# peabody124/PosePipeline

Measured on AMD Instinct MI355X. Metric: frames/sec (whole node), detect->2D->3D cascade on 1080p; MPJPE vs reference, higher is better.
Workload: dtype f32; eligible float32 convolutions are evaluated as 2-term float16 splits (22 significand bits under per-channel / per-sample power-of-two scales, 3 products per term) on the 16-bit matrix cores with float32 accumulation (float32-accurate at any input magnitude, not bit-identical: tests/test_gpu_spl

## Files before the change

### include/posepipe_hip.h

```cpp
#ifndef POSEPIPE_HIP_H
#define POSEPIPE_HIP_H

#include <stddef.h>
#include <stdint.h>

#ifdef __cplusplus
extern "C" {
#endif

#define PP_ABI_VERSION 10

typedef enum {
    PP_OK = 0,
    PP_ERR_ARG = -1,
    PP_ERR_HIP = -2,
    PP_ERR_STATE = -3,
    PP_ERR_UNSUPPORTED = -4
} pp_status;

typedef enum { PP_MEM_HOST = 0, PP_MEM_DEVICE = 1 } pp_mem_kind;

typedef struct pp_ctx pp_ctx;
typedef struct pp_net pp_net;
typedef struct pp_tracker pp_tracker;
// ... 70 lines not shown
    int32_t up2_log2, up3_log2;
} pp_op;

typedef struct pp_buf {
    int32_t h, w, c;
    int32_t pad;
} pp_buf;

int pp_net_create(pp_ctx* ctx, const pp_op* ops, int n_ops, const pp_buf* bufs, int n_bufs,
                  const float* weights, size_t n_weights, int max_batch, pp_net** out);
int pp_net_create_mem(pp_ctx* ctx, const pp_op* ops, int n_ops, const pp_buf* bufs, int n_bufs,
                      const float* weights, size_t n_weights, int weights_mem, int max_batch, pp_net** out);
#define PP_NET_NUMERICS_DEFAULT 0
#define PP_NET_NUMERICS_EXACT 1
#define PP_NET_NUMERICS_SPLIT 2
#define PP_NET_NUMERICS_SPLIT_BF16 3
#define PP_NET_NUMERICS_SPLIT_F16 4
int pp_net_create_ex(pp_ctx* ctx, const pp_op* ops, int n_ops, const pp_buf* bufs, int n_bufs,
                     const float* weights, size_t n_weights, int weights_mem, int max_batch, int numerics, pp_net** out);
int pp_net_numerics(pp_net* net);
int pp_net_split_kind(pp_net* net);
void pp_net_destroy(pp_net* net);
int pp_net_buffer(pp_net* net, int buf, void** dptr, size_t* bytes_per_sample);
int pp_net_input_amax(pp_net* net, int buf, void** dptr);
int pp_net_run(pp_net* net, int batch, int first_op, int last_op);
int pp_net_forward(pp_net* net, int batch, int in_buf, const float* in, int out_buf, float* out,
                   int mem);
int pp_net_set_lanes(pp_net* net, int enable);
int pp_net_set_lane_count(pp_net* net, int n_lanes);
int pp_net_capture(pp_net* net, int batch);
int pp_net_profile(pp_net* net, int batch, float* ms_per_op);
int pp_net_conv_kinds(pp_net* net, int* kinds);
int pp_net_folded_into(pp_net* net, int* into);

int pp_conv_force(int ct, int pt);
int pp_conv_variant(int variant);
int pp_conv_exact(int exact);
int pp_conv_split_kind(int f16);

int pp_conv2d(pp_ctx* ctx, const pp_op* op, int n, int hin, int win, const float* x,
              const float* w, const float* bias, const float* res1, const float* res2, float* y,
              int res1_h, int res1_w, int mem);

int pp_crop_resize_bilinear(pp_ctx* ctx, const float* src_nhwc4, int n_src, int src_h, int src_w, const int32_t* rects5, int n,
                            int out_h, int out_w, float* out_nhwc4);

int pp_net_vit_timing(pp_net* net, int enable, float* ms3, int* n_gemm);
int pp_f32_to_bf16(pp_ctx* ctx, const float* x, uint16_t* y, size_t n);
int pp_gemm_bf16(pp_ctx* ctx, const uint16_t* a, const uint16_t* w, const float* bias, const float* res, int res_mod,
                 void* c, int m, int n, int k, int act, int out_bf16);
int pp_layernorm(pp_ctx* ctx, const float* x, const float* gamma, const float* beta, int rows, int dim, float eps,
                 void* y, int out_bf16);
int pp_attention_bf16(pp_ctx* ctx, const uint16_t* qkv, int batch, int tokens, int heads, int head_dim, uint16_t* out);

int pp_crop_affine_normalize(pp_ctx* ctx, const uint8_t* frames, int n_frames, int h, int w,
                             const int32_t* frame_idx, const double* bbox_tlwh, int n_person,
                             int out_w, int out_h, const float* lut, const int32_t* chan_map,
                             int flip, float* out, float* center_scale, uint8_t* crop_u8,
                             int32_t* valid, int mem);

int pp_flip_merge_decode(pp_ctx* ctx, const float* hm, const float* hm_flip, int n, int k, int h,
                         int w, const int32_t* flip_perm, int shift_heatmap, int post,
                         int blur_kernel, const float* center_scale, float* kpts, float* merged,
                         int mem);

int pp_topdown_create(pp_net* net, int in_buf, int out_buf, int num_joints, const int32_t* flip_perm,
// ... 136 lines not shown
```

### posepipeline_amd/csrc/conv_split.hip

```cpp
#include <algorithm>
#include <atomic>
#include <map>
#include <mutex>
#include <type_traits>
#include <vector>
#include <cstring>
#include <cstdio>

#include "pp_internal.h"
#include "pp_amax.h"

#ifndef PP_SPLIT_ABLATE
#define PP_SPLIT_ABLATE 0
#endif

typedef __attribute__((ext_vector_type(8))) __bf16 bf16x8;
typedef __attribute__((ext_vector_type(8))) _Float16 f16x8;
typedef __attribute__((ext_vector_type(16))) float f32x16;

std::atomic<int> g_split_gemm_epi{-1};

namespace {


struct SplitArgs {
    const float* x;
    const uint4* w;
    const float* bias;
    const float* res1;
    const float* res2;
    float* y;
    int N, H, W, Cin, Cout, ncb;
    int xp_h, xp_w;
    int y_pad, r1_pad, r2_pad, relu;
    int nchunks;
    int tiles_x, tiles_y, TH, TW, bw_log2, gx_log2;
    int PWp;
    int NP, NPp;
    int mode, stride;
    int r1_shift, r1_H, r1_W;
    int ktaps, KW, pad, Hin, Win;
    long long S;
    unsigned x_bytes;
    int xcd_remap;
    int SP;
    int gx, gy;
    int col_major;
    int epi_lds;
    unsigned dv_per[2], dv_row[2];
    unsigned dv_tx[2], dv_ty[2], dv_pw[2];
    unsigned dv_ncol[2], dv_run0[2], dv_run1[2];
    unsigned dv_ktaps[2], dv_kw[2];
    const float* wscale;
    const unsigned* x_amax;
    unsigned* y_amax;
    const float* x2;
    const unsigned* x2_amax;
    int Cin2, stride2, xp2_h, xp2_w, seg1;
#ifdef PP_SPLIT_TIMELINE
    unsigned long long* dbg;
#endif
};

#ifdef PP_SPLIT_TIMELINE
#define PP_TL_DECL unsigned long long tl_t[10] = {0, 0, 0, 0, 0, 0, 0, 0, 0, 0}
#define PP_TL_MARK(i) do { if (a.dbg) tl_t[i] = __builtin_amdgcn_s_memtime(); } while (0)
#define PP_TL_FLUSH()                                                                                                    \
    do {                                                                                                                 \
        if (a.dbg && threadIdx.x == 0) {                                                                                 \
            unsigned hw, xcc;                                                                                            \
            asm volatile("s_getreg_b32 %0, hwreg(HW_REG_HW_ID)" : "=s"(hw));                                            \
            asm volatile("s_getreg_b32 %0, hwreg(HW_REG_XCC_ID)" : "=s"(xcc));                                          \
            unsigned long long* r = a.dbg + (size_t)blockIdx.x * 16;                                                     \
            r[0] = blockIdx.x; r[1] = ((unsigned long long)xcc << 32) | hw;                                              \
            r[2] = tl_t[0]; r[3] = tl_t[1]; r[4] = tl_t[2]; r[5] = tl_t[3]; r[6] = L; r[7] = col;                       \
            for (int i_ = 4; i_ < 10; ++i_) r[4 + i_] = tl_t[i_];                                                        \
        }                                                                                                                \
    } while (0)
#else
#define PP_TL_DECL
#define PP_TL_MARK(i)
#define PP_TL_FLUSH()
// ... 60 lines not shown
        if (x > 20.f) return x;
        const double n = exp((double)x);
        const double t = n * (n + 2.0);
        return x * (float)(t / (t + 2.0));
    }
    if (act == PP_ACT_ELU) return x > 0.f ? x : (float)expm1((double)x);
    if (act == PP_ACT_SWISH) return x * (float)(1.0 / (1.0 + exp(-(double)x)));
    return x;
}

__device__ __forceinline__ int lane_q(int r) {
    const int g1 = ((r >= 4 && r < 12) || (r >= 16 && r < 20) || r >= 28) ? 1 : 0;
    int idx;
    if (!g1) idx = r < 4 ? r : r < 16 ? r - 8 : r - 12;
    else idx = r < 12 ? r - 4 : r < 20 ? r - 8 : r - 16;
    return g1 * 16 + idx;
}
__device__ __forceinline__ void block_pixel(int r, int bw_log2, int& iy, int& ix) {
    if (bw_log2 == 0) {
        iy = 0;
        ix = r;
        return;
    }
    const int q = lane_q(r);
    if (bw_log2 == 1) {
        iy = q >> 4;
        ix = q & 15;
    } else {
        iy = ((q >> 3) & 1) * 2 + (q >> 4);
        ix = q & 7;
    }
}

enum { MODE_TILE = 0, MODE_STREAM = 1, MODE_GEMM = 2 };

template <int T, int NSLOT, int COB, int PXB = 2, int NW = 4, bool RING4 = false, bool H = false, bool S2 = false>
__global__ __launch_bounds__(64 * NW, NW == 4 ? 2 : 1) void conv_split_kernel(SplitArgs a) {
    static_assert(!S2 || (T == 9 && RING4 && H && PXB == 1), "S2 is the 4-wave fp16 ring form with one pixel block per wave");
    constexpr int NT = 64 * NW;
    constexpr int XP = H ? 2 : 3;
    constexpr int WPL = H ? 2 : 3;
    constexpr bool WLDS = NW == 8 || RING4;
    static_assert(!RING4 || (NW == 4 && T == 9), "RING4 is the 4-wave 3x3 form");
    extern __shared__ __attribute__((aligned(16))) unsigned char smem[];
    const int tid = threadIdx.x;
    const int lane = tid & 63;
    const int wave = tid >> 6;
    unsigned L = blockIdx.x, col = blockIdx.y;
    PP_TL_DECL;
    PP_TL_MARK(0);
    if (a.xcd_remap) {
        if (!xcd_tile_column(blockIdx.x, a, L, col)) return;
    }
    const int cb0 = (int)col * COB;
    const int plane_bytes = 2 * a.NPp * 16;
    const int buf_bytes = XP * plane_bytes;

    int n = 0, x0 = 0, y0 = 0;
    unsigned s0 = 0;
    if (a.mode == MODE_TILE) {
        const unsigned L2 = pp_udiv(L, a.dv_tx);
        const int tx = (int)(L - L2 * (unsigned)a.tiles_x);
        n = (int)pp_udiv(L2, a.dv_ty);
        const int ty = (int)(L2 - (unsigned)n * (unsigned)a.tiles_y);
        x0 = tx * a.TW;
        y0 = ty * a.TH;
    } else {
        s0 = L * (unsigned)(32 * PXB * NW);
    }

    unsigned goff[NSLOT];
    unsigned vmask[T == 1 ? NSLOT : 1];
    int simg[H ? NSLOT : 1];
    const int woff0 = ((((tid & 3) >> 1) * a.NPp + (tid >> 2)) * 16 + (tid & 1) * 8);
    if (a.mode == MODE_STREAM) {
        const int pos0 = (int)s0 - a.PWp - 1 + (tid >> 2);
        const unsigned cin4 = (unsigned)a.Cin * 4u;
        const unsigned base = (unsigned)pos0 * cin4 + (unsigned)(tid & 3) * 16u;
#pragma unroll
        for (int j = 0; j < NSLOT; ++j) goff[j] = pos0 + (NT / 4) * j < 0 ? 0xffffffffu : base + (unsigned)((NT / 4) * j) * cin4;
        if constexpr (T == 1) {
#pragma unroll
            for (int j = 0; j < NSLOT; ++j) vmask[j] = 0;
        }
        if constexpr (H) {
#pragma unroll
            for (int j = 0; j < NSLOT; ++j) {
                const int pj = pos0 + (NT / 4) * j;
                simg[j] = (int)pp_udiv((unsigned)min(max(pj, 0), (int)a.S - 1), a.dv_per);
            }
        }
    } else {
#pragma unroll
    for (int j = 0; j < NSLOT; ++j) {
        const int u = tid + NT * j;
        const int p = u >> 2, quad = u & 3;
        const bool in_patch = p < a.NP;
        unsigned off = 0xffffffffu;
        if constexpr (H) simg[j] = n;
        if constexpr (S2) {
            const int ph = (int)pp_udiv((unsigned)p, a.dv_row), r = p - ph * a.SP;
            const int qr = (int)pp_udiv((unsigned)r, a.dv_pw), qc = r - qr * a.PWp;
            const int pr = 2 * qr + (ph >> 1), pc = 2 * qc + (ph & 1);
            const int iy = 2 * y0 - 1 + pr, ix = 2 * x0 - 1 + pc;
            if (in_patch && pc <= 2 * a.TW && (unsigned)iy < (unsigned)a.Hin && (unsigned)ix < (unsigned)a.Win)
                off = (unsigned)(((n * a.xp_h + iy) * a.xp_w + ix) * a.Cin) * 4u;
        } else if (a.mode == MODE_TILE) {
            const int pr = (int)pp_udiv((unsigned)p, a.dv_pw), pc = p - pr * a.PWp;
            const int iy = y0 - 1 + pr, ix = x0 - 1 + pc;
            if (in_patch && pc < a.TW + 2 && (unsigned)iy < (unsigned)a.H && (unsigned)ix < (unsigned)a.W)
                off = (unsigned)(((n * a.xp_h + iy) * a.xp_w + ix) * a.Cin) * 4u;
        } else {
            const unsigned m = s0 + (unsigned)p;
            if constexpr (T == 1) vmask[j] = 0;
            if (in_patch && m < (unsigned)a.S) {
                const int img = (int)pp_udiv(m, a.dv_per), rem = (int)(m - (unsigned)img * (unsigned)(a.H * a.W));
                const int ho = (int)pp_udiv((unsigned)rem, a.dv_row), wo = rem - ho * a.W;
                if constexpr (H) simg[j] = img;
                if (T == 1 && a.ktaps > 1) {
                    const int iy0 = ho * a.stride - a.pad, ix0 = wo * a.stride - a.pad;
                    off = (unsigned)(((img * a.xp_h + iy0) * a.xp_w + ix0) * a.Cin) * 4u;
                    unsigned vm = 0;
// ... 80 lines not shown
    if constexpr (WLDS) {
        issue_w(0);
        issue_w(1);
        issue_w(2);
        load_patch(0);
    } else {
        load_patch(0);
        load_w(wf[0]);
    }
    unsigned xam[H ? NSLOT : 1];
    if constexpr (H) {
#pragma unroll
        for (int j = 0; j < NSLOT; ++j) xam[j] = a.x_amax[simg[j]];
    }
    __builtin_amdgcn_sched_barrier(0);

    auto pixel_coords = [&](int lane_, int wave_, int pb, int& aofs_, int& on_, int& oy_, int& ox_, bool& ok_) {
        if (a.mode == MODE_TILE) {
            const int BW = 32 >> a.bw_log2, BH = 1 << a.bw_log2;
            int by, bx;
            block_pixel(lane_ & 31, a.bw_log2, by, bx);
            const int b = wave_ * PXB + pb;
            const int gy = b >> a.gx_log2, gx = b & ((1 << a.gx_log2) - 1);
            const int ry = gy * BH + by, rx = gx * BW + bx;
            aofs_ = (((lane_ >> 5) * a.NPp) + ry * a.PWp + rx) * 16;
            on_ = n;
            oy_ = y0 + ry;
            ox_ = x0 + rx;
            ok_ = oy_ < a.H && ox_ < a.W;
        } else {
            const unsigned per = a.mode == MODE_STREAM ? (unsigned)(a.xp_h * a.PWp) : (unsigned)(a.H * a.W);
            const unsigned row = a.mode == MODE_STREAM ? (unsigned)a.PWp : (unsigned)a.W;
            const int pl = (wave_ * PXB + pb) * 32 + (lane_ & 31);
            aofs_ = (((lane_ >> 5) * a.NPp) + pl) * 16;
            const unsigned sp = s0 + (unsigned)pl;
            const bool in = sp < (unsigned)a.S;
            const unsigned sc = in ? sp : 0u;
            const unsigned img = pp_udiv(sc, a.dv_per);
            const unsigned rem = sc - img * per;
            const unsigned yy = pp_udiv(rem, a.dv_row);
            on_ = (int)img;
            oy_ = (int)yy;
            ox_ = (int)(rem - yy * row);
            ok_ = in && oy_ < a.H && ox_ < a.W;
        }
    };
    int aofs[PXB];
#pragma unroll
    for (int pb = 0; pb < PXB; ++pb) {
        int on_, oy_, ox_;
        bool ok_;
        pixel_coords(lane, wave, pb, aofs[pb], on_, oy_, ox_, ok_);
    }

    f32x16 acc[COB][PXB];
#pragma unroll
    for (int cb = 0; cb < COB; ++cb)
#pragma unroll
        for (int pb = 0; pb < PXB; ++pb)
#pragma unroll
            for (int i = 0; i < 16; ++i) acc[cb][pb][i] = 0.f;
    if constexpr (H) {
#pragma unroll
        for (int q = 0; q < (NSLOT + 3) / 4; ++q) sxe[q] = 0;
#pragma unroll
        for (int j = 0; j < NSLOT; ++j) sxe[j >> 2] |= pp_amax_exp(xam[j]) << (8 * (j & 3));
    }

    auto load_x = [&](const unsigned char* pbuf, int t, int pb) {
        const int dy = t / 3, dx = t % 3;
        const int toff = S2 ? ((((dy & 1) * 2 + (dx & 1)) * a.SP) + (dy >> 1) * a.PWp + (dx >> 1)) * 16 : T == 9 ? (dy * a.PWp + dx) * 16 : 0;
#pragma unroll
        for (int pl = 0; pl < XP; ++pl) xf[pb][pl] = *reinterpret_cast<const uint4*>(pbuf + pl * plane_bytes + aofs[pb] + toff);
    };

    if constexpr (!WLDS) {
        store_patch(0, 0, NSLOT);
// ... 1525 lines not shown
}

__global__ __launch_bounds__(256) void split_weights_stem7_kernel(const float* w, uint4* out, int CoutPad, const float* cmax) {
    const int i = blockIdx.x * 256 + threadIdx.x;
    if (i >= STEM_STEPS * 2 * 64) return;
    const int lane = i & 63, cb = (i >> 6) & 1, s = i >> 7;
    const int cout = cb * 32 + (lane & 31);
    unsigned short h[2][8];
#pragma unroll
    for (int j = 0; j < 8; ++j) {
        const int dy = s >> 1, dx = 4 * (s & 1) + 2 * (lane >> 5) + (j >> 2), c = j & 3;
        float v = 0.f;
        if (dx < 7) {
            const int k = (dy * 7 + dx) * 4 + c;
            v = w[((size_t)(k >> 5) * CoutPad + cout) * 32 + 8 * (k & 3) + ((k & 31) >> 2)];
        }
        unsigned short q2;
        split_weight_h(v, channel_scale(cmax[cout]), h[0][j], h[1][j], q2);
    }
#pragma unroll
    for (int pn = 0; pn < 2; ++pn) {
        uint4 o;
        o.x = h[pn][0] | ((unsigned)h[pn][1] << 16);
        o.y = h[pn][2] | ((unsigned)h[pn][3] << 16);
        o.z = h[pn][4] | ((unsigned)h[pn][5] << 16);
        o.w = h[pn][6] | ((unsigned)h[pn][7] << 16);
        out[(size_t)(((s * 2 + cb) * 2 + pn) * 64 + lane)] = o;
    }
}

}


static TileGeom tap_tiling(const ConvArgs& a, int nw, int stream_env) {
    const int max_np = nw == 8 ? 768 : 512, xp_h = a.Hin + a.x_pad, xp_w = a.Win + a.x_pad;
    TileGeom g = pick_tile(a.Hout, a.Wout, max_np, nw / 2);
    g.mode = MODE_TILE;
    const int snp = 64 * nw + 2 + 2 * xp_w;
    const double stream_eff = (double)a.Hout * a.Wout / ((double)xp_h * xp_w);
    bool use_stream = a.x_pad >= 1 && snp <= max_np && (g.eff < 0 || stream_eff > g.eff + 0.02);
    if (stream_env == 0 && g.eff >= 0) use_stream = false;
    if (stream_env == 1 && a.x_pad >= 1 && snp <= max_np) use_stream = true;
    if (use_stream) {
        g.mode = MODE_STREAM;
        g.PWp = xp_w;
        g.NP = g.NPp = snp;
        while (g.NPp % 8 != 4) ++g.NPp;
    }
    return g;
}

SplitPlan pp_conv_split_plan(const ConvArgs& a) {
    static const int stem7_on = env_int("POSEPIPE_SPLIT_STEM7", 1);
    static const int s2_on = env_int("POSEPIPE_SPLIT_S2", 1), s2p_on = env_int("POSEPIPE_SPLIT_S2P", 1);
    static const int gemm8_on = env_int("POSEPIPE_SPLIT_GEMM8", 1), gemm4_min_c = env_int("POSEPIPE_SPLIT_GEMM4_MIN_C", 64);
    static const int gemm_min_cin = env_int("POSEPIPE_SPLIT_GEMM_MIN_CIN", 1024);
    static const int c48_on = env_int("POSEPIPE_SPLIT_C48", 1), c48_mult = env_int("POSEPIPE_SPLIT_C48_MULT", 0);
    static const int stream_env = env_int("POSEPIPE_SPLIT_STREAM", -1);
    const char* s2_env = getenv("POSEPIPE_SPLIT_S2_MIN_CIN");
    SplitPlan p;
    p.f16 = a.split_f16 != 0;
    const size_t wpl = p.f16 ? 2 : 3;
    p.ncb = (a.Cout + 31) / 32;
    p.nout = p.ncb * 32;
    if (stem7_on && p.f16 && a.KH == 7 && a.KW == 7 && a.stride == 2 && a.pad_h == 3 && a.pad_w == 3 && a.dil_h == 1 && a.dil_w == 1 &&
        a.Cin == 4 && a.Cout == 64 && a.CoutPad >= 64 && a.up_log2 == 0 && !a.out_nchw && !a.res1 && !a.res2 &&
        (a.relu == PP_RELU_NONE || a.relu == PP_RELU_FIRST || a.relu == PP_RELU_LAST) && (a.y_stride == 0 || a.y_stride == a.Cout) &&
        a.y_coff == 0 && a.Hout == (a.Hin - 1) / 2 + 1 && a.Wout == (a.Win - 1) / 2 + 1) {
        p.kernel = SPLIT_STEM7;
        p.cin = a.Cin;
        p.frag_bytes = STEM_WBYTES;
        p.bytes = p.frag_bytes + (size_t)2 * p.nout * sizeof(float);
        return p;
    }
    const bool k3 = a.KH == 3 && a.KW == 3 && a.stride == 1 && a.pad_h == 1 && a.pad_w == 1 && a.dil_h == 1 && a.dil_w == 1 &&
                    a.Hout == a.Hin && a.Wout == a.Win;
    const bool k1 = a.KH == 1 && a.KW == 1 && a.pad_h == 0 && a.pad_w == 0;
    const bool full = a.KH == a.Hin && a.KW == a.Win && a.pad_h == 0 && a.pad_w == 0 && a.dil_h == 1 && a.dil_w == 1 &&
                      a.x_pad == 0 && a.Hout == 1 && a.Wout == 1 && !k1;
    const bool s2_pick = s2_env ? a.Cin >= atoi(s2_env) : p.f16 ? (a.Cin >= 96 || (a.Cin >= 48 && p.ncb >= 6)) : (a.Cin >= 128 && (p.ncb & 1) == 0);
    const bool s2_shape = a.KH == 3 && a.KW == 3 && a.stride == 2 && a.pad_h == 1 && a.pad_w == 1 && a.dil_h == 1 && a.dil_w == 1 && !full;
    const bool s2p_map = a.Hout * a.Wout >= 1500 || (a.Hout * a.Wout >= 400 && a.Cout >= 96);
    const bool s2p = s2p_on && p.f16 && s2_shape && s2p_map;
    const bool k3s2 = s2_on && s2_shape && (s2_pick || s2p);
    if (!(k3 || k1 || full || k3s2)) return p;
    p.taps = (k3 || k3s2) ? 9 : 1;
    p.cin = full ? a.K : a.Cin;
    const bool product = gemm8_on && p.taps == 1 && p.cin >= gemm4_min_c && a.Cout % 128 == 0;
    const bool one_column = p.f16 && p.cin >= 256 && a.Cout > 32 && a.Cout <= 64 && a.HWout >= 4096;
    if (p.taps == 1 && p.cin < gemm_min_cin && !one_column && !product) return p;
    const bool res1_plain = !a.res1 || (a.res1_off_w == 0 && a.res1_shift >= 0 && a.res1_shift <= 4 &&
                                        ((a.Hout - 1) >> a.res1_shift) < a.res1_H && ((a.Wout - 1) >> a.res1_shift) < a.res1_W &&
                                        (a.res1_shift > 0 || (a.res1_H == a.Hout && a.res1_W == a.Wout)));
    if (!(p.cin % 16 == 0 && a.Cout % 4 == 0 && a.up_log2 == 0 && !a.out_nchw && res1_plain && a.relu <= PP_ACT_SWISH &&
          (a.y_stride == 0 || a.y_stride == a.Cout) && a.y_coff == 0))
        return p;
    const bool c48 = c48_on && k3 && ((a.Cout > 32 && a.Cout <= 48) || (c48_mult == 1 && a.Cout % 48 == 0) || (c48_mult == 2 && a.Cout == 192));
    if (a.Cin2 > 0) {
        if (!(product && p.f16 && k1 && a.stride == 1 && !a.res1 && a.Cin2 % 16 == 0 && a.stride2 >= 1 && a.x_pad == 0 && a.x2_pad == 0 &&
              (a.Hout - 1) * a.stride2 < a.Hin2 && (a.Wout - 1) * a.stride2 < a.Win2))
            return SplitPlan();
        p.cin2 = a.Cin2;
    }
    size_t steps = (size_t)((p.cin + p.cin2) / 16) * p.taps;
    if (product) {
        p.kernel = SPLIT_PRODUCT;
    } else if (!k3 && !s2p) {
        p.kernel = p.taps > 1 ? SPLIT_TAP_GATHER : SPLIT_ONE_TAP;
        p.tile[0].mode = MODE_GEMM;
        p.tile[0].NP = 256;
        p.tile[0].NPp = 260;
    } else if (s2p) {
        p.kernel = SPLIT_S2P;
        p.tile[0] = pick_tile_s2(a.Hout, a.Wout, 13 * 64);
        p.tile[0].mode = MODE_TILE;
    } else if (c48) {
        p.kernel = SPLIT_C48;
        p.ncb = (a.Cout + 47) / 48 * 3;
        p.nout = p.ncb * 16;
        steps = (size_t)(p.cin / 16) * 5;
        p.tile[0] = tap_tiling(a, 4, stream_env);
    } else {
        p.kernel = SPLIT_TAP3;
        p.tile[0] = tap_tiling(a, 4, stream_env);
        p.tile[1] = tap_tiling(a, 8, stream_env);
    }
    p.frag_bytes = (steps + 1) * p.ncb * wpl * 64 * sizeof(uint4);
    p.bytes = p.frag_bytes + (p.f16 ? (size_t)2 * p.nout * sizeof(float) : 0);
    if (p.cin2 > 0) {
        p.bias_off = (p.bytes + 15) / 16 * 16;
        p.bytes = p.bias_off + (size_t)a.CoutPad * sizeof(float);
    }
    return p;
}

static int split_weights_folded(const SplitPlan& p, const ConvArgs& a, void* out, hipStream_t stream) {
    const int kcat = p.cin + p.cin2, kpad = (kcat + 31) / 32 * 32;
    const size_t total = (size_t)kpad * a.CoutPad;
    float* cat = nullptr;
    PP_HIP_CHECK(hipMalloc((void**)&cat, total * sizeof(float)));
    hipLaunchKernelGGL(concat_weights_kernel, dim3((unsigned)((total + 255) / 256)), dim3(256), 0, stream, a.w, a.w2, cat, p.cin, p.cin2, a.CoutPad, total);
    SplitPlan q = p;
    q.cin = kcat;
    q.cin2 = 0;
    ConvArgs b = a;
    b.w = cat;
    b.Cin = kcat; b.K = kcat; b.Kpad = kpad;
    int rc = pp_conv_split_weights(q, b, out, stream);
    std::vector<float> b0(a.CoutPad), b1(a.CoutPad);
    hipError_t e = hipStreamSynchronize(stream);
    if (e == hipSuccess) e = hipMemcpy(b0.data(), a.bias, b0.size() * sizeof(float), hipMemcpyDeviceToHost);
    if (e == hipSuccess) e = hipMemcpy(b1.data(), a.bias2, b1.size() * sizeof(float), hipMemcpyDeviceToHost);
    for (size_t i = 0; i < b0.size(); ++i) b0[i] += b1[i];
    if (e == hipSuccess) e = hipMemcpy(static_cast<unsigned char*>(out) + p.bias_off, b0.data(), b0.size() * sizeof(float), hipMemcpyHostToDevice);
    (void)hipFree(cat);
    if (rc == PP_OK && e != hipSuccess) {
        pp_set_error("split_weights (folded shortcut) failed: %s", hipGetErrorString(e));
// ... 73 lines not shown
    if (!path || (only_cin && a.Cin != only_cin) || recorded >= max_launches) return nullptr;
    ++recorded;
    if (!tl_buf && hipMalloc(&tl_buf, TL_MAX_WG * 128) != hipSuccess) return nullptr;
    (void)hipMemsetAsync(tl_buf, 0, TL_MAX_WG * 128, stream);
    return tl_buf;
}
static void tl_end(const ConvArgs& a, const SplitArgs& s, const char* kernel, unsigned nwg, hipStream_t stream) {
    if (!s.dbg) return;
    (void)hipStreamSynchronize(stream);
    nwg = std::min<unsigned>(nwg, TL_MAX_WG);
    std::vector<unsigned long long> h((size_t)nwg * 16);
    (void)hipMemcpy(h.data(), tl_buf, h.size() * 8, hipMemcpyDeviceToHost);
    static int launch = 0;
    FILE* f = fopen(getenv("POSEPIPE_SPLIT_TIMELINE"), "ab");
    if (!f) return;
    long long hdr[16] = {0x54494d454c494e45ll, launch++, (long long)nwg, a.N, a.Hout, a.Wout, a.Cin, a.Cout, s.mode, s.nchunks, s.gx, s.gy,
                         a.res1 != nullptr, a.res2 != nullptr, 0, 0};
    memcpy(&hdr[14], kernel, std::min<size_t>(strlen(kernel), 15));
    fwrite(hdr, 8, 16, f);
    fwrite(h.data(), 8, h.size(), f);
    fclose(f);
}
#define PP_TL_BEGIN() s.dbg = tl_begin(a, stream)
#define PP_TL_END(name, nwg) tl_end(a, s, name, nwg, stream)
#else
#define PP_TL_BEGIN()
#define PP_TL_END(name, nwg)
#endif

static void fill_divisors(SplitArgs& s) {
    const bool stream_mode = s.mode == MODE_STREAM;
    make_magic(stream_mode ? (unsigned)(s.xp_h * s.PWp) : (unsigned)(s.H * s.W), s.dv_per);
    make_magic(stream_mode ? (unsigned)s.PWp : (unsigned)s.W, s.dv_row);
    make_magic((unsigned)std::max(s.tiles_x, 1), s.dv_tx);
    make_magic((unsigned)std::max(s.tiles_y, 1), s.dv_ty);
    make_magic((unsigned)std::max(s.PWp, 1), s.dv_pw);
    make_magic((unsigned)std::max(s.gy, 1), s.dv_ncol);
    make_magic((unsigned)std::max(s.gx >> 3, 1), s.dv_run0);
    make_magic((unsigned)((s.gx >> 3) + 1), s.dv_run1);
    make_magic((unsigned)std::max(s.ktaps, 1), s.dv_ktaps);
    make_magic((unsigned)std::max(s.KW, 1), s.dv_kw);
}

template <auto K, int MAX_LDS, class Args>
static void launch_split(dim3 grid, unsigned threads, size_t lds, hipStream_t stream, const Args& s) {
    static PpPerDeviceOnce once;
    once.run([] { (void)hipFuncSetAttribute((const void*)K, hipFuncAttributeMaxDynamicSharedMemorySize, MAX_LDS); });
    hipLaunchKernelGGL(K, grid, dim3(threads), lds, stream, s);
}

template <int NS, int... MORE, class F>
static void with_nslot(int nslot, F&& f) {
    if constexpr (sizeof...(MORE) == 0) f(std::integral_constant<int, NS>());
    else if (nslot <= NS) f(std::integral_constant<int, NS>());
    else with_nslot<MORE...>(nslot, f);
}

template <int T, int NW, bool R4, int NS>
static void launch_tap(int cob, bool f16, dim3 grid, size_t lds, hipStream_t stream, const SplitArgs& s) {
    constexpr int L = (NW == 8 ? 160 : 100) * 1024;
    if constexpr (R4) {
        if (cob == 3) return launch_split<conv_split_kernel<9, NS, 3, 2, 4, true, true>, L>(grid, 256, lds, stream, s);
        if (cob == 4) return launch_split<conv_split_kernel<9, NS, 4, 2, 4, true, true>, L>(grid, 256, lds, stream, s);
    }
    if (f16 && cob == 2) launch_split<conv_split_kernel<T, NS, 2, 2, NW, R4, true>, L>(grid, 64 * NW, lds, stream, s);
    else if (f16) launch_split<conv_split_kernel<T, NS, 1, 2, NW, R4, true>, L>(grid, 64 * NW, lds, stream, s);
    else if (cob == 2) launch_split<conv_split_kernel<T, NS, 2, 2, NW, R4, false>, L>(grid, 64 * NW, lds, stream, s);
    else launch_split<conv_split_kernel<T, NS, 1, 2, NW, R4, false>, L>(grid, 64 * NW, lds, stream, s);
}

static unsigned apply_tiling(SplitArgs& s, const TileGeom& g, const ConvArgs& a, int nw) {
    s.mode = g.mode;
    s.NP = g.NP;
    s.NPp = g.NPp;
    if (g.mode == MODE_GEMM) {
        s.S = (long long)a.M;
        return (unsigned)((a.M + 255) / 256);
    }
    s.PWp = g.PWp;
    if (g.mode == MODE_STREAM) {
        s.S = (long long)a.N * s.xp_h * s.xp_w;
        return (unsigned)((s.S + 64 * nw - 1) / (64 * nw));
    }
    s.tiles_x = g.tiles_x; s.tiles_y = g.tiles_y; s.TH = g.TH; s.TW = g.TW; s.bw_log2 = g.bw_log2; s.gx_log2 = g.gx_log2;
    return (unsigned)(g.tiles_x * g.tiles_y * a.N);
}

static int launch_stem7(const ConvArgs& a, hipStream_t stream) {
    if (!a.x_amax) {
        pp_set_error("conv_split: the fp16 form needs the per-sample maximum of its input (ConvArgs::x_amax)");
        return PP_ERR_STATE;
    }
    StemArgs s{};
    s.x = a.x; s.w = (const uint4*)a.wsplit; s.bias = a.bias; s.y = a.y;
    s.wscale = reinterpret_cast<const float*>(static_cast<const unsigned char*>(a.wsplit) + STEM_WBYTES);
    s.x_amax = a.x_amax; s.y_amax = a.y_amax;
    s.N = a.N; s.Hin = a.Hin; s.Win = a.Win; s.xp_h = a.Hin + a.x_pad; s.xp_w = a.Win + a.x_pad;
    s.Hout = a.Hout; s.Wout = a.Wout; s.y_pad = a.y_pad; s.relu = a.relu;
    s.tiles_x = (a.Wout + STEM_TW - 1) / STEM_TW;
    s.tiles_y = (a.Hout + STEM_TH - 1) / STEM_TH;
    s.ntiles = a.N * s.tiles_x * s.tiles_y;
    s.x_bytes = a.x_bytes;
    make_magic((unsigned)s.tiles_x, s.dv_tx);
    make_magic((unsigned)s.tiles_y, s.dv_ty);
    static const int ncu = [] {
        int dev = 0, n = 256;
        if (hipGetDevice(&dev) == hipSuccess) (void)hipDeviceGetAttribute(&n, hipDeviceAttributeMultiprocessorCount, dev);
        return n > 0 ? n : 256;
    }();
    launch_split<conv_split_stem7_kernel, STEM_LDS>(dim3((unsigned)std::min(s.ntiles, ncu)), 512, STEM_LDS, stream, s);
    hipError_t e = hipGetLastError();
    if (e != hipSuccess) {
        pp_set_error("conv_split_stem7 launch failed: %s", hipGetErrorString(e));
        return PP_ERR_HIP;
    }
    return PP_OK;
}

int pp_launch_conv_split(const SplitPlan& p, const ConvArgs& a, hipStream_t stream) {
    if (a.wsplit && p.kernel == SPLIT_STEM7) return launch_stem7(a, stream);
    if (!a.wsplit || p.kernel == SPLIT_NONE) {
        pp_set_error("conv_split: layer not eligible");
        return PP_ERR_ARG;
    }
    static const int colmaj_mb = env_int("POSEPIPE_SPLIT_COLMAJOR_MB", 256), gemm_remap = env_int("POSEPIPE_SPLIT_GEMM_REMAP", 1);
    static const int epi_env = env_int("POSEPIPE_SPLIT_GEMM_EPI", 1);
    static const int cob2_env = env_int("POSEPIPE_SPLIT_S2_COB", 0), cob_env = env_int("POSEPIPE_SPLIT_COB", 0);
    static const int nw8_f16 = env_int("POSEPIPE_SPLIT_NW8_F16", 0);
    static const int nw8_min_blocks = env_int("POSEPIPE_SPLIT_NW8_MIN_BLOCKS", 512), nw8_min_chunks = env_int("POSEPIPE_SPLIT_NW8_MIN_CHUNKS", 16);
    static const int ring4_env = env_int("POSEPIPE_SPLIT_RING4", 1), ring48_env = env_int("POSEPIPE_SPLIT_RING48", 1);
    const bool full = p.cin != a.Cin;
    SplitArgs s{};
    s.x = a.x; s.w = (const uint4*)a.wsplit; s.bias = a.bias; s.res1 = a.res1; s.res2 = a.res2; s.y = a.y;
    s.N = a.N; s.H = a.Hout; s.W = a.Wout; s.Cin = p.cin; s.Cout = a.Cout;
    s.ncb = p.ncb;
    s.xp_h = full ? 1 : a.Hin + a.x_pad;
    s.xp_w = full ? 1 : a.Win + a.x_pad;
    s.stride = a.stride;
    s.y_pad = a.y_pad; s.r1_pad = a.r1_pad; s.r2_pad = a.r2_pad; s.relu = a.relu;
    s.r1_shift = a.res1 ? a.res1_shift : 0;
    s.r1_H = a.res1 ? a.res1_H : a.Hout;
    s.r1_W = a.res1 ? a.res1_W : a.Wout;
    s.nchunks = (p.cin + p.cin2) / 16;
// ... 74 lines not shown
        });
        tag = "s2p";
    } else if (p.kernel == SPLIT_C48) {
        const unsigned gx = apply_tiling(s, p.tile[0], a, 4);
        s.gx = (int)gx;
        s.gy = s.ncb / 3;
        grid = s.xcd_remap ? dim3((unsigned)((s.gx + 7) / 8 * 8 * s.gy), 1) : dim3(gx, (unsigned)s.gy);
        fill_divisors(s);
        const size_t patch48 = (size_t)2 * xp * 2 * s.NPp * 16;
        const bool ring48 = f16 && ring48_env && patch48 + (size_t)4 * 3 * wpl * 1024 <= 80 * 1024;
        const size_t lds = patch48 + (ring48 ? (size_t)4 * 3 * wpl * 1024 : 0);
        with_nslot<5, 6, 7, 8>((s.NP + 63) / 64, [&](auto ns) {
            constexpr int NS = decltype(ns)::value, L = 100 * 1024;
            if (ring48) launch_split<conv_split48_kernel<NS, true, true>, L>(grid, 256, lds, stream, s);
            else if (f16) launch_split<conv_split48_kernel<NS, true, false>, L>(grid, 256, lds, stream, s);
            else launch_split<conv_split48_kernel<NS, false, false>, L>(grid, 256, lds, stream, s);
        });
        tag = "c48";
    } else {
        const bool tap3 = p.kernel == SPLIT_TAP3;
        int cob = (s.ncb & 1) ? 1 : 2;
        if (tap3 && f16 && s.ncb % 3 == 0 && (cob_env == 0 || cob_env == 3)) cob = 3;
        else if (tap3 && f16 && s.ncb % 4 == 0 && (cob_env == 0 || cob_env == 4)) cob = 4;
        int nw = tap3 && (!f16 || nw8_f16) ? 8 : 4;
        unsigned gx = apply_tiling(s, p.tile[nw == 8], a, nw);
        if (nw == 8 && !((long)gx * (s.ncb / cob) >= nw8_min_blocks && s.nchunks >= nw8_min_chunks)) {
            nw = 4;
            gx = apply_tiling(s, p.tile[0], a, nw);
        }
        const int nslot = (s.NP + 16 * nw - 1) / (16 * nw);
        const auto ring_fits = [&](int c) {
            return ring4_env && nw == 4 && s.mode != MODE_GEMM && (size_t)xp * 2 * s.NPp * 16 + (size_t)4 * c * wpl * 1024 <= 80 * 1024;
        };
        if (cob >= 3 && !(ring_fits(cob) && (cob_env >= 3 || (long)gx * (s.ncb / cob) >= 400))) cob = (s.ncb & 1) ? 1 : 2;
        const bool ring = ring_fits(cob);
        grid = dim3(gx, (unsigned)(s.ncb / cob));
        s.gx = (int)grid.x; s.gy = (int)grid.y;
        if (s.xcd_remap) grid = dim3((unsigned)((s.gx + 7) / 8 * 8 * s.gy), 1);
        const size_t lds = (size_t)(ring ? 1 : 2) * xp * 2 * s.NPp * 16 + ((nw == 8 || ring) ? (size_t)4 * cob * wpl * 1024 : 0);
        fill_divisors(s);
        if (s.mode == MODE_GEMM) launch_tap<1, 4, false, 4>(cob, f16, grid, lds, stream, s);
        else if (nw == 8) with_nslot<5, 6>(nslot, [&](auto ns) { launch_tap<9, 8, false, decltype(ns)::value>(cob, f16, grid, lds, stream, s); });
        else if (ring) with_nslot<5, 6, 7, 8>(nslot, [&](auto ns) { launch_tap<9, 4, true, decltype(ns)::value>(cob, f16, grid, lds, stream, s); });
        else with_nslot<5, 6, 7, 8>(nslot, [&](auto ns) { launch_tap<9, 4, false, decltype(ns)::value>(cob, f16, grid, lds, stream, s); });
        tag = s.mode == MODE_GEMM ? "gemm4" : nw == 8 ? "nw8" : ring ? "ring4" : "nw4";
    }
    PP_TL_END(tag, grid.x * grid.y);
    hipError_t e = hipGetLastError();
    if (e != hipSuccess) {
        pp_set_error("conv_split (%s) launch failed: %s", tag, hipGetErrorString(e));
        return PP_ERR_HIP;
    }
    return PP_OK;
}
```

### posepipeline_amd/csrc/net.hip

```cpp
#include <algorithm>
#include <memory>

#include "pp_internal.h"
#include "pp_amax.h"

struct pp_net {
    pp_ctx* ctx = nullptr;
    std::vector<pp_op> ops;
    std::vector<pp_buf> bufs;
    std::vector<size_t> buf_off;
    std::vector<size_t> buf_elems;
    float* weights = nullptr;
    size_t n_weights = 0;
    unsigned char* wsplit = nullptr;
    std::vector<SplitPlan> split_plan;
    int numerics = PP_NET_NUMERICS_EXACT;
    int split_f16 = 0;
    unsigned* amax = nullptr;
    std::vector<int> op_x_slot, op_y_slot, op_post_slot, slot_owner;
    std::vector<int> op_x2_slot;
    std::vector<int> fold_into, fold_src;
    bool folded(int i) const { return !fold_into.empty() && fold_into[i] >= 0; }
    int carries(int i) const { return fold_src.empty() ? -1 : fold_src[i]; }
    void reads(int i, int (&r)[5]) const {
// ... 867 lines not shown
            if (net->op_needs_event[i]) PP_HIP_CHECK(hipEventCreateWithFlags(&net->op_done[i], hipEventDisableTiming));
        PP_HIP_CHECK(hipEventCreateWithFlags(&net->fork_ev, hipEventDisableTiming));
        net->join_ev.resize(n_lanes);
        for (auto& e : net->join_ev) PP_HIP_CHECK(hipEventCreateWithFlags(&e, hipEventDisableTiming));
    }
    return PP_OK;
}

int pp_net_input_amax(pp_net* net, int buf, void** dptr) {
    PP_REQUIRE(net && dptr && buf >= 0 && buf < (int)net->bufs.size(), "pp_net_input_amax: bad argument");
    *dptr = nullptr;
    for (auto& e : net->ext)
        if (e.buf == buf && net->amax) {
            e.provided = true;
            *dptr = net->amax_slot(e.slot);
        }
    return PP_OK;
}

int pp_net_conv_kinds(pp_net* net, int* kinds) {
    PP_REQUIRE(net && kinds, "pp_net_conv_kinds: NULL argument");
    for (size_t i = 0; i < net->ops.size(); ++i) {
        kinds[i] = net->ops[i].type != PP_OP_CONV ? 0 : net->split_plan[i].kernel != SPLIT_NONE || net->folded((int)i) ? 2 : 1;
    }
    return PP_OK;
}

int pp_net_folded_into(pp_net* net, int* into) {
    PP_REQUIRE(net && into, "pp_net_folded_into: NULL argument");
    for (size_t i = 0; i < net->ops.size(); ++i) into[i] = net->folded((int)i) ? net->fold_into[i] : -1;
    return PP_OK;
}

void pp_net_destroy(pp_net* net) { delete net; }

int pp_net_buffer(pp_net* net, int buf, void** dptr, size_t* bytes_per_sample) {
    PP_REQUIRE(net && buf >= 0 && buf < (int)net->bufs.size(), "pp_net_buffer: bad buffer id");
    PP_REQUIRE(net->bufs[buf].pad == 0, "pp_net_buffer: buffer %d has a zero halo (conv-internal layout); expose dense buffers only", buf);
    if (dptr) *dptr = net->buf_ptr(buf);
    if (bytes_per_sample) *bytes_per_sample = net->buf_elems[buf] * sizeof(float);
    return PP_OK;
}

int pp_net_run(pp_net* net, int batch, int first_op, int last_op) {
    PP_REQUIRE(net, "pp_net_run: net is NULL");
    PP_REQUIRE(batch > 0 && batch <= net->max_batch, "pp_net_run: batch %d not in (0,%d]", batch, net->max_batch);
    if (last_op < 0) last_op = (int)net->ops.size();
    PP_REQUIRE(first_op >= 0 && last_op <= (int)net->ops.size() && first_op <= last_op, "pp_net_run: bad op range");
    if (net->graph_exec && batch == net->graph_batch && first_op == 0 && last_op == (int)net->ops.size()) {
        PP_HIP_CHECK(hipGraphLaunch(net->graph_exec, net->ctx->stream));
        for (auto& e : net->ext) e.provided = false;
        return PP_OK;
    }
    hipStream_t main = net->ctx->stream;
    PpRange range("pp_net_run");
    PP_TRY(net_reset_amax(net, first_op, last_op, batch, main));
    if (net->lanes.empty() || !net->use_lanes || last_op - first_op < 8) {
        for (int i = first_op; i < last_op; ++i) PP_TRY(net_launch_op(net, i, batch, main));
        return PP_OK;
    }
    PP_HIP_CHECK(hipEventRecord(net->fork_ev, main));
    for (hipStream_t l : net->lanes) PP_HIP_CHECK(hipStreamWaitEvent(l, net->fork_ev, 0));
    for (int i = first_op; i < last_op; ++i) {
        hipStream_t s = net->lanes[net->op_lane[i]];
        for (int d : net->op_waits[i])
            if (d >= first_op) PP_HIP_CHECK(hipStreamWaitEvent(s, net->op_done[d], 0));
// ... 117 lines not shown
```

Measured before the change: 619.9.

## Add dense output-pixel mode for 3x3 fp16 split convolutions

Adds a MODE_DENSE tiling for the 4-wave 3x3 split-conv kernel. Each workgroup covers a contiguous run of real output pixels and maps them back to padded-input stream offsets, so no lanes are spent on halo positions the way stream mode spends them. It is chosen for fp16 splits when stream mode's useful-pixel share is below a threshold, and it allows cob=3 when the grid fits within the CU count. The cost is extra index arithmetic per pixel and a larger input patch footprint in LDS. It also adds a query API that reports which tap mode each conv uses.

```diff
diff --git a/include/posepipe_hip.h b/include/posepipe_hip.h
--- a/include/posepipe_hip.h
+++ b/include/posepipe_hip.h
@@ -126,6 +126,7 @@
 int pp_net_profile(pp_net* net, int batch, float* ms_per_op);
 int pp_net_conv_kinds(pp_net* net, int* kinds);
 int pp_net_folded_into(pp_net* net, int* into);
+int pp_net_tap_modes(pp_net* net, int* modes);
 
 int pp_conv_force(int ct, int pt);
 int pp_conv_variant(int variant);
diff --git a/posepipeline_amd/csrc/conv_split.hip b/posepipeline_amd/csrc/conv_split.hip
--- a/posepipeline_amd/csrc/conv_split.hip
+++ b/posepipeline_amd/csrc/conv_split.hip
@@ -48,6 +48,7 @@
     int col_major;
     int epi_lds;
     unsigned dv_per[2], dv_row[2];
+    unsigned dv_sper[2];
     unsigned dv_tx[2], dv_ty[2], dv_pw[2];
     unsigned dv_ncol[2], dv_run0[2], dv_run1[2];
     unsigned dv_ktaps[2], dv_kw[2];
@@ -174,7 +175,7 @@
     }
 }
 
-enum { MODE_TILE = 0, MODE_STREAM = 1, MODE_GEMM = 2 };
+enum { MODE_TILE = 0, MODE_STREAM = 1, MODE_GEMM = 2, MODE_DENSE = 3 };
 
 template <int T, int NSLOT, int COB, int PXB = 2, int NW = 4, bool RING4 = false, bool H = false, bool S2 = false>
 __global__ __launch_bounds__(64 * NW, NW == 4 ? 2 : 1) void conv_split_kernel(SplitArgs a) {
@@ -210,13 +211,19 @@
     } else {
         s0 = L * (unsigned)(32 * PXB * NW);
     }
+    unsigned sp0 = s0;
+    if (a.mode == MODE_DENSE) {
+        const unsigned img = pp_udiv(s0, a.dv_per), rem = s0 - img * (unsigned)(a.H * a.W);
+        const unsigned yy = pp_udiv(rem, a.dv_row);
+        sp0 = img * (unsigned)(a.xp_h * a.PWp) + yy * (unsigned)a.PWp + (rem - yy * (unsigned)a.W);
+    }
 
     unsigned goff[NSLOT];
     unsigned vmask[T == 1 ? NSLOT : 1];
     int simg[H ? NSLOT : 1];
     const int woff0 = ((((tid & 3) >> 1) * a.NPp + (tid >> 2)) * 16 + (tid & 1) * 8);
-    if (a.mode == MODE_STREAM) {
-        const int pos0 = (int)s0 - a.PWp - 1 + (tid >> 2);
+    if (a.mode == MODE_STREAM || a.mode == MODE_DENSE) {
+        const int pos0 = (int)sp0 - a.PWp - 1 + (tid >> 2);
         const unsigned cin4 = (unsigned)a.Cin * 4u;
         const unsigned base = (unsigned)pos0 * cin4 + (unsigned)(tid & 3) * 16u;
 #pragma unroll
@@ -226,10 +233,11 @@
             for (int j = 0; j < NSLOT; ++j) vmask[j] = 0;
         }
         if constexpr (H) {
+            const int slast = a.N * a.xp_h * a.PWp - 1;
 #pragma unroll
             for (int j = 0; j < NSLOT; ++j) {
                 const int pj = pos0 + (NT / 4) * j;
-                simg[j] = (int)pp_udiv((unsigned)min(max(pj, 0), (int)a.S - 1), a.dv_per);
+                simg[j] = (int)pp_udiv((unsigned)min(max(pj, 0), slast), a.dv_sper);
             }
         }
     } else {
@@ -376,7 +384,6 @@
             const unsigned per = a.mode == MODE_STREAM ? (unsigned)(a.xp_h * a.PWp) : (unsigned)(a.H * a.W);
             const unsigned row = a.mode == MODE_STREAM ? (unsigned)a.PWp : (unsigned)a.W;
             const int pl = (wave_ * PXB + pb) * 32 + (lane_ & 31);
-            aofs_ = (((lane_ >> 5) * a.NPp) + pl) * 16;
             const unsigned sp = s0 + (unsigned)pl;
             const bool in = sp < (unsigned)a.S;
             const unsigned sc = in ? sp : 0u;
@@ -387,6 +394,9 @@
             oy_ = (int)yy;
             ox_ = (int)(rem - yy * row);
             ok_ = in && oy_ < a.H && ox_ < a.W;
+            int pp = pl;
+            if (a.mode == MODE_DENSE && in) pp = (int)(img * (unsigned)(a.xp_h * a.PWp) + yy * (unsigned)a.PWp) + ox_ - (int)sp0;
+            aofs_ = (((lane_ >> 5) * a.NPp) + pp) * 16;
         }
     };
     int aofs[PXB];
@@ -1978,7 +1988,8 @@
 }
 
 
-static TileGeom tap_tiling(const ConvArgs& a, int nw, int stream_env) {
+static const double DENSE_MAX_SHARE = 0.85;
+static TileGeom tap_tiling(const ConvArgs& a, int nw, int stream_env, int dense_env = -2) {
     const int max_np = nw == 8 ? 768 : 512, xp_h = a.Hin + a.x_pad, xp_w = a.Win + a.x_pad;
     TileGeom g = pick_tile(a.Hout, a.Wout, max_np, nw / 2);
     g.mode = MODE_TILE;
@@ -1993,6 +2004,16 @@
         g.NP = g.NPp = snp;
         while (g.NPp % 8 != 4) ++g.NPp;
     }
+    if (dense_env >= -1 && dense_env != 0 && a.x_pad >= 1) {
+        const int P = 64 * nw, HW = a.Hout * a.Wout;
+        const int dnp = (P - 1) + a.x_pad * ((P - 1 + a.Wout - 1) / a.Wout) + a.x_pad * xp_w * ((P - 1 + HW - 1) / HW) + 1 + 2 * xp_w + 2;
+        if (dnp <= max_np && (dense_env == 1 || (use_stream && stream_eff < DENSE_MAX_SHARE))) {
+            g.mode = MODE_DENSE;
+            g.PWp = xp_w;
+            g.NP = g.NPp = dnp;
+            while (g.NPp % 8 != 4) ++g.NPp;
+        }
+    }
     return g;
 }
 
@@ -2004,6 +2025,8 @@
     static const int c48_on = env_int("POSEPIPE_SPLIT_C48", 1), c48_mult = env_int("POSEPIPE_SPLIT_C48_MULT", 0);
     static const int stream_env = env_int("POSEPIPE_SPLIT_STREAM", -1);
     const char* s2_env = getenv("POSEPIPE_SPLIT_S2_MIN_CIN");
+    const char* dense_s = getenv("POSEPIPE_SPLIT_DENSE");
+    const int dense_env = dense_s ? std::max(-1, std::min(1, atoi(dense_s))) : -1;
     SplitPlan p;
     p.f16 = a.split_f16 != 0;
     const size_t wpl = p.f16 ? 2 : 3;
@@ -2068,7 +2091,7 @@
         p.tile[0] = tap_tiling(a, 4, stream_env);
     } else {
         p.kernel = SPLIT_TAP3;
-        p.tile[0] = tap_tiling(a, 4, stream_env);
+        p.tile[0] = tap_tiling(a, 4, stream_env, p.f16 ? dense_env : -2);
         p.tile[1] = tap_tiling(a, 8, stream_env);
     }
     p.frag_bytes = (steps + 1) * p.ncb * wpl * 64 * sizeof(uint4);
@@ -2208,6 +2231,7 @@
     const bool stream_mode = s.mode == MODE_STREAM;
     make_magic(stream_mode ? (unsigned)(s.xp_h * s.PWp) : (unsigned)(s.H * s.W), s.dv_per);
     make_magic(stream_mode ? (unsigned)s.PWp : (unsigned)s.W, s.dv_row);
+    make_magic((unsigned)std::max(s.xp_h * s.PWp, 1), s.dv_sper);
     make_magic((unsigned)std::max(s.tiles_x, 1), s.dv_tx);
     make_magic((unsigned)std::max(s.tiles_y, 1), s.dv_ty);
     make_magic((unsigned)std::max(s.PWp, 1), s.dv_pw);
@@ -2254,12 +2278,25 @@
         return (unsigned)((a.M + 255) / 256);
     }
     s.PWp = g.PWp;
+    if (g.mode == MODE_DENSE) {
+        s.S = (long long)a.N * a.Hout * a.Wout;
+        return (unsigned)((s.S + 64 * nw - 1) / (64 * nw));
+    }
     if (g.mode == MODE_STREAM) {
         s.S = (long long)a.N * s.xp_h * s.xp_w;
         return (unsigned)((s.S + 64 * nw - 1) / (64 * nw));
     }
     s.tiles_x = g.tiles_x; s.tiles_y = g.tiles_y; s.TH = g.TH; s.TW = g.TW; s.bw_log2 = g.bw_log2; s.gx_log2 = g.gx_log2;
     return (unsigned)(g.tiles_x * g.tiles_y * a.N);
+}
+
+static int device_cus() {
+    static const int ncu = [] {
+        int dev = 0, n = 256;
+        if (hipGetDevice(&dev) == hipSuccess) (void)hipDeviceGetAttribute(&n, hipDeviceAttributeMultiprocessorCount, dev);
+        return n > 0 ? n : 256;
+    }();
+    return ncu;
 }
 
 static int launch_stem7(const ConvArgs& a, hipStream_t stream) {
@@ -2279,12 +2316,7 @@
     s.x_bytes = a.x_bytes;
     make_magic((unsigned)s.tiles_x, s.dv_tx);
     make_magic((unsigned)s.tiles_y, s.dv_ty);
-    static const int ncu = [] {
-        int dev = 0, n = 256;
-        if (hipGetDevice(&dev) == hipSuccess) (void)hipDeviceGetAttribute(&n, hipDeviceAttributeMultiprocessorCount, dev);
-        return n > 0 ? n : 256;
-    }();
-    launch_split<conv_split_stem7_kernel, STEM_LDS>(dim3((unsigned)std::min(s.ntiles, ncu)), 512, STEM_LDS, stream, s);
+    launch_split<conv_split_stem7_kernel, STEM_LDS>(dim3((unsigned)std::min(s.ntiles, device_cus())), 512, STEM_LDS, stream, s);
     hipError_t e = hipGetLastError();
     if (e != hipSuccess) {
         pp_set_error("conv_split_stem7 launch failed: %s", hipGetErrorString(e));
@@ -2425,7 +2457,9 @@
         const auto ring_fits = [&](int c) {
             return ring4_env && nw == 4 && s.mode != MODE_GEMM && (size_t)xp * 2 * s.NPp * 16 + (size_t)4 * c * wpl * 1024 <= 80 * 1024;
         };
-        if (cob >= 3 && !(ring_fits(cob) && (cob_env >= 3 || (long)gx * (s.ncb / cob) >= 400))) cob = (s.ncb & 1) ? 1 : 2;
+        const long wg3 = (long)gx * (s.ncb / cob);
+        const bool own_cu = s.mode == MODE_DENSE && cob == 3 && wg3 <= device_cus() && (long)gx * (s.ncb / ((s.ncb & 1) ? 1 : 2)) > device_cus();
+        if (cob >= 3 && !(ring_fits(cob) && (cob_env >= 3 || wg3 >= 400 || own_cu))) cob = (s.ncb & 1) ? 1 : 2;
         const bool ring = ring_fits(cob);
         grid = dim3(gx, (unsigned)(s.ncb / cob));
         s.gx = (int)grid.x; s.gy = (int)grid.y;
@@ -2436,7 +2470,7 @@
         else if (nw == 8) with_nslot<5, 6>(nslot, [&](auto ns) { launch_tap<9, 8, false, decltype(ns)::value>(cob, f16, grid, lds, stream, s); });
         else if (ring) with_nslot<5, 6, 7, 8>(nslot, [&](auto ns) { launch_tap<9, 4, true, decltype(ns)::value>(cob, f16, grid, lds, stream, s); });
         else with_nslot<5, 6, 7, 8>(nslot, [&](auto ns) { launch_tap<9, 4, false, decltype(ns)::value>(cob, f16, grid, lds, stream, s); });
-        tag = s.mode == MODE_GEMM ? "gemm4" : nw == 8 ? "nw8" : ring ? "ring4" : "nw4";
+        tag = s.mode == MODE_GEMM ? "gemm4" : nw == 8 ? "nw8" : s.mode == MODE_DENSE ? (ring ? "ring4d" : "nw4d") : ring ? "ring4" : "nw4";
     }
     PP_TL_END(tag, grid.x * grid.y);
     hipError_t e = hipGetLastError();
diff --git a/posepipeline_amd/csrc/net.hip b/posepipeline_amd/csrc/net.hip
--- a/posepipeline_amd/csrc/net.hip
+++ b/posepipeline_amd/csrc/net.hip
@@ -923,6 +923,13 @@
     return PP_OK;
 }
 
+int pp_net_tap_modes(pp_net* net, int* modes) {
+    PP_REQUIRE(net && modes, "pp_net_tap_modes: NULL argument");
+    for (size_t i = 0; i < net->ops.size(); ++i)
+        modes[i] = net->ops[i].type == PP_OP_CONV && net->split_plan[i].kernel == SPLIT_TAP3 ? net->split_plan[i].tile[0].mode : -1;
+    return PP_OK;
+}
+
 void pp_net_destroy(pp_net* net) { delete net; }
 
 int pp_net_buffer(pp_net* net, int buf, void** dptr, size_t* bytes_per_sample) {
```

Result: no change. 623.1 (median of 6 runs) (+0.5%).
